# trailofbits/reverie

Measured on AMD Instinct MI355X. Metric: prover AND-gates/sec on GF(2) Bristol circuit; 1/2/4/8-GPU; proof bit-exact, higher is better.
Workload: dtype u32; 1 GPU; synthetic layered AND/XOR GF(2) circuit, 10027008 gates (5014185 AND), 4096 inputs, 153 layers x 65536, p_and=0.5, 256 reps x 8 players, 40 online; parallelism=reps/1, levels=163, compile_hint=RV_COMPILE_WHOLE_PROVER, gate_stream_bytes=334698564

## Files before the change

reverie_amd/csrc/gf2dev.h:

```cpp
#pragma once
#include <hip/hip_runtime.h>
#include <stdint.h>

namespace rv {

__device__ __forceinline__ uint32_t smear01(uint32_t t) {
    uint32_t r;
    asm("v_lshlrev_b32 %0, 8, %1\n\tv_sub_u32 %0, %0, %1" : "=&v"(r) : "v"(t));
    return r;
}
__device__ __forceinline__ uint32_t recon32(uint32_t t) {
    t ^= t >> 4;
    t ^= t >> 2;
    t ^= t >> 1;
    t &= 0x01010101u;
    return smear01(t);
}

__device__ __forceinline__ uint32_t expand4(uint32_t n) {
    const uint32_t t = (n | (n << 7) | (n << 14) | (n << 21)) & 0x01010101u;
    return smear01(t);
}
__device__ __forceinline__ uint32_t compress4(uint32_t x) {
    const uint32_t y = x & 0x08040201u;
    return (y | (y >> 8) | (y >> 16) | (y >> 24)) & 0xFu;
}
__device__ __forceinline__ uint32_t load_bits(const uint8_t* base, size_t row, uint32_t NQ, uint32_t q) {
    return expand4(((uint32_t)base[row * (NQ >> 1) + (q >> 1)] >> (4 * (q & 1))) & 0xFu);
}
__device__ __forceinline__ uint32_t pair_swap(uint32_t v) {
    return (uint32_t)__builtin_amdgcn_mov_dpp((int)v, 0xB1, 0xF, 0xF, true);
}
__device__ __forceinline__ void store_bits(uint8_t* base, size_t row, uint32_t NQ, uint32_t q, uint32_t smeared) {
    const uint32_t n = compress4(smeared);
    const uint32_t other = pair_swap(n);
    if (!(q & 1)) base[row * (NQ >> 1) + (q >> 1)] = (uint8_t)(n | (other << 4));
}

}
```

reverie_amd/csrc/internal.h:

```cpp
#pragma once
#include <hip/hip_runtime.h>
#include <stddef.h>
#include <stdint.h>

#include "../../include/reverie_amd.h"

namespace rv {


constexpr int RV_LIN_K = 3;
struct Gate {
    uint32_t op;
    uint32_t dst;
    uint32_t m;
    uint32_t eo;
    uint32_t ep;
    uint32_t x;
    uint32_t a[RV_LIN_K], b[RV_LIN_K];
};

enum GateOp : uint32_t {
    G_INPUT = 0,
    G_XORK,
    G_MUL,
// ... 14 lines not shown
    uint32_t m;
    uint32_t m2;
    uint64_t eo;
    uint64_t ep;
    uint32_t x;
    uint32_t xc;
    uint64_t imm;
    uint32_t am, bm;
};
constexpr uint32_t G64_MASK_ROW = 0x80000000u;

enum Gate64Op : uint32_t {
    G64_INPUT = 0, G64_ADD, G64_SUB, G64_ADDC, G64_SUBC, G64_MULC, G64_MUL, G64_ASSERT, G64_RANDOM, G64_CONST, G64_B2A
};

struct Interp64Params {
    uint32_t R;
    uint64_t* wmask;
    uint64_t* wcorr;
    const uint64_t* masks;
    uint64_t* on;
    uint64_t* pre;
    uint64_t on_words, pre_words;
    const uint64_t* wit;
    const uint8_t* omit;
    const uint64_t* sup_in;
    const uint64_t* sup_corr;
    const uint64_t* sup_rec;
    uint32_t sup_r;
    const uint8_t* corr2;
    const uint32_t* masks2;
    uint32_t NQ;
    int* err;
};

enum Mode : int { MODE_PROVE = 0, MODE_VERIFY = 1, MODE_PROVE_V = 2,  MODE_VERIFY_C = 4 };
constexpr int RV_DEV_ZERO_CHECK = 0x100;

struct InterpParams {
    uint32_t NQ;
    uint32_t* rows;
    uint8_t* corr;
    uint32_t* on;
    uint8_t* pre;
    uint8_t* vclr;
    uint64_t* vc;
    const uint8_t* wit;
    const uint32_t* on_mask;
    const uint32_t* sup_in;
    const uint32_t* sup_corr;
    const uint32_t* sup_rec;
    uint32_t sup_nq;
    int* err;
};

void set_device_lds_limit(size_t bytes);
size_t device_lds_limit();

struct EvalParams {
    uint32_t B, W;
    uint32_t* val;
    const uint32_t* win;
    uint64_t* v64;
    const uint64_t* wz;
    uint64_t wz_stride;
    uint32_t* n_failed;
    uint32_t* first2;
    uint32_t* first64;
};
struct WireForm {
    uint32_t b[RV_LIN_K];
    uint32_t c;
};
void launch_eval_level(hipStream_t st, const EvalParams& p, const Gate* d_gates, uint32_t lo, uint32_t n2, const Gate64* d_gates64, uint32_t lo64,
                       uint32_t n64);
struct LevelRange;
void launch_eval_walk(hipStream_t st, const EvalParams& p, const Gate* d_gates, const LevelRange* d_lr, const Gate64* d_gates64, const uint32_t* d_ls64,
                      uint32_t n_levels, uint32_t S, uint32_t threads);
void launch_eval_wit(hipStream_t st, const uint8_t* d_wit , uint32_t n, uint32_t B, uint32_t W, uint32_t* d_out );
void launch_eval_out(hipStream_t st, const EvalParams& p, const WireForm* d_forms, uint32_t n_gf2, const uint32_t* d_ssa64, uint32_t n_z64,
                     uint8_t* d_out2 , uint64_t* d_out64 );

struct EvalFold {
    const uint32_t* rec2;
    const uint64_t* op2;
    const uint32_t* rec64;
    const uint64_t* op64;
    uint32_t n2, n64;
    uint64_t op_base;
    uint64_t* first_op;
    uint64_t* total;
};
void launch_eval_fold(hipStream_t st, const EvalParams& p, const EvalFold& f);
void launch_eval_stream_out(hipStream_t st, const EvalParams& p, uint32_t n_gf2, uint32_t n_z64, uint32_t b0, uint32_t nb, uint8_t* d_out2,
                            uint64_t* d_out64);

void launch_expand_seeds(hipStream_t st, const uint8_t* d_seeds, uint32_t n_reps, uint8_t* d_keys );
constexpr uint32_t RK_BYTES = 208;
constexpr uint32_t RK_AREAS = 13;
constexpr uint64_t RV_MAX_CTR_BLOCKS = 1ull << 24;
void launch_key_schedule(hipStream_t st, const uint8_t* d_keys, uint32_t n_slots, uint8_t* d_rkbytes );
void launch_setup_keys(hipStream_t st, const uint8_t* d_seeds, uint32_t NQ, uint8_t* d_keys, uint8_t* d_rkbytes, uint32_t* d_rk, uint32_t* d_img);
void launch_bitslice_rk(hipStream_t st, const uint8_t* d_rkbytes, uint32_t NQ, uint32_t* d_rk );
void launch_aes_gf2_masks(hipStream_t st, const uint32_t* d_rk, const uint32_t* d_keep, uint32_t NQ, uint64_t first_block,
                          uint64_t n_blocks, uint32_t* d_masks);
bool aes_col4_supports(uint32_t NQ);
// ... 150 lines not shown
```

reverie_amd/csrc/kernels.hip:

```cpp
#include <stdlib.h>

#include <algorithm>

#include "b3.h"
#include "gf2dev.h"
#include "internal.h"
#include "launch.h"

namespace rv {

static size_t g_device_lds_limit = 160 * 1024;
void set_device_lds_limit(size_t bytes) { g_device_lds_limit = bytes; }
size_t device_lds_limit() { return g_device_lds_limit; }


__device__ __forceinline__ uint32_t gather_rows(const uint32_t* rows, const uint32_t* ids, uint32_t NQ, uint32_t q) {
    uint32_t v = 0;
#pragma unroll
    for (int i = 0; i < RV_LIN_K; i++) v ^= rows[(size_t)ids[i] * NQ + q];
    return v;
}
__device__ __forceinline__ uint32_t gather_corr_byte(const uint8_t* corr, const uint32_t* ids, uint32_t NQ, uint32_t o) {
    uint32_t v = 0;
#pragma unroll
// ... 26 lines not shown
    v |= (uint32_t)__builtin_amdgcn_update_dpp(0, (int)v, 0x111, 0xF, 0xF, true);
    v |= (uint32_t)__builtin_amdgcn_update_dpp(0, (int)v, 0x112, 0xF, 0xF, true);
    v |= (uint32_t)__builtin_amdgcn_update_dpp(0, (int)v, 0x114, 0xF, 0xF, true);
    if (q == 7 || q == 15) ((uint32_t*)(vc + row))[q >> 3] = v;
}
constexpr bool is_verify(int mode) { return mode == MODE_VERIFY || mode == MODE_VERIFY_C; }

#ifndef RV_COH_LDROW
#define RV_COH_LDROW 1
#endif
#ifndef RV_COH_STROW
#define RV_COH_STROW 1
#endif
#ifndef RV_COH_V
#define RV_COH_V 1
#endif
template <int COH>
__device__ __forceinline__ uint32_t ld_row(const uint32_t* p) {
    if (COH && RV_COH_LDROW) return __hip_atomic_load(const_cast<uint32_t*>(p), __ATOMIC_RELAXED, __HIP_MEMORY_SCOPE_AGENT);
    return *p;
}
template <int COH>
__device__ __forceinline__ void st_row(uint32_t* p, uint32_t v) {
    if (COH == 1 && RV_COH_STROW)
        __hip_atomic_store(p, v, __ATOMIC_RELAXED, __HIP_MEMORY_SCOPE_AGENT);
    else
        *p = v;
}
template <int COH>
__device__ __forceinline__ uint32_t ld_v(const uint8_t* p) {
    if (COH && RV_COH_V) return __hip_atomic_load(const_cast<uint8_t*>(p), __ATOMIC_RELAXED, __HIP_MEMORY_SCOPE_AGENT);
    return *p;
}
template <int COH>
__device__ __forceinline__ void st_v(uint8_t* p, uint8_t v) {
    if (COH == 1 && RV_COH_V)
        __hip_atomic_store(p, v, __ATOMIC_RELAXED, __HIP_MEMORY_SCOPE_AGENT);
    else
        *p = v;
}
template <int COH>
__device__ __forceinline__ uint32_t gather_rows_c(const uint32_t* rows, const uint32_t* ids, uint32_t NQ, uint32_t q) {
    uint32_t v = 0;
#pragma unroll
    for (int i = 0; i < RV_LIN_K; i++) v ^= ld_row<COH>(&rows[(size_t)ids[i] * NQ + q]);
    return v;
}
template <int COH>
__device__ __forceinline__ uint32_t gather_vclr_c(const uint8_t* vclr, const uint32_t* ids) {
    uint32_t v = 0;
#pragma unroll
    for (int i = 0; i < RV_LIN_K; i++) v ^= ld_v<COH>(&vclr[ids[i]]);
    return v;
}

template <int MODE, int COH = 0>
__device__ __forceinline__ void interp_one_impl(const Gate& g, const InterpParams& p, uint32_t NQ, uint32_t q, uint32_t onm) {
    switch (g_op(g)) {
    case G_INPUT: {
        const uint32_t lam = p.rows[(size_t)g.m * NQ + q];
        uint32_t corr;
        if (!is_verify(MODE)) {
            const uint32_t w = p.wit[g.x] ? 0xFFFFFFFFu : 0u;
            corr = w ^ recon32(lam);
        } else {
            corr = onm ? (p.sup_in[(size_t)g.x * p.sup_nq + q] & onm) : 0u;
        }
        if (!is_verify(MODE) || onm) p.on[(size_t)g.eo * NQ + q] = corr;
        if (MODE == MODE_PROVE_V) {
            if (q == 0) st_v<COH>(&p.vclr[g.dst], p.wit[g.x] ? 1 : 0);
        } else if (MODE == MODE_VERIFY_C) {
            vc_store(p.vc, g.dst, q, corr);
        } else {
            store_bits(p.corr, g.dst, NQ, q, corr);
        }
        break;
    }
    case G_XORK: {
        st_row<COH>(&p.rows[(size_t)g.dst * NQ + q], gather_rows_c<COH>(p.rows, g.a, NQ, q) ^ gather_rows_c<COH>(p.rows, g.b, NQ, q));
        if (MODE == MODE_PROVE_V) {
            if (q == 0) st_v<COH>(&p.vclr[g.dst], (uint8_t)((g_ca(g) ^ gather_vclr_c<COH>(p.vclr, g.a) ^ gather_vclr_c<COH>(p.vclr, g.b)) & 1u));
            break;
        }
        if (MODE == MODE_VERIFY_C) {
            if (q == 0) p.vc[g.dst] = gather_vc(p.vc, g.a) ^ gather_vc(p.vc, g.b) ^ (g_ca(g) ? ~0ull : 0ull);
            break;
        }
        if (!(q & 1)) {
            const size_t h = NQ >> 1, o = q >> 1;
            const uint32_t c = (g_ca(g) ? 0xFFu : 0u) ^ gather_corr_byte(p.corr, g.a, NQ, o) ^ gather_corr_byte(p.corr, g.b, NQ, o);
            p.corr[(size_t)g.dst * h + o] = (uint8_t)c;
        }
        break;
    }
    case G_RANDOM: {
        if (MODE == MODE_VERIFY_C) {
            if (q == 0) p.vc[g.dst] = 0;
            break;
        }
        if (!(q & 1)) p.corr[(size_t)g.dst * (NQ >> 1) + (q >> 1)] = 0;
        break;
    }
    case G_MUL: {
        const uint32_t lx = gather_rows_c<COH>(p.rows, g.a, NQ, q), ly = gather_rows_c<COH>(p.rows, g.b, NQ, q);
        const uint32_t lab = p.rows[(size_t)g.m * NQ + q], lnew = p.rows[(size_t)(g.m + 1) * NQ + q];
        const uint32_t a = recon32(lx), b = recon32(ly), c = recon32(lab);
// ... 80 lines not shown
}

#ifndef RV_B3_RPL
#define RV_B3_RPL 4
#endif
#ifndef RV_INTERP_UNROLL
#define RV_INTERP_UNROLL 4
#endif
#ifndef RV_INTERP_UNROLL_SMALL
#define RV_INTERP_UNROLL_SMALL 2
#endif
#ifndef RV_INTERP_UNROLL_MID
#define RV_INTERP_UNROLL_MID 4
#endif
#ifndef RV_INTERP_UNROLL_FAST
#define RV_INTERP_UNROLL_FAST 4
#endif
#ifndef RV_INTERP_UXOR_FAST
#define RV_INTERP_UXOR_FAST 0
#endif
__host__ __device__ constexpr int interp_unroll(int NQ, bool general = true) {
    return NQ >= 64 ? (general ? RV_INTERP_UNROLL : RV_INTERP_UNROLL_FAST) : NQ >= 32 ? RV_INTERP_UNROLL_MID : RV_INTERP_UNROLL_SMALL;
}

struct PfPlan {
    uint32_t dist;
    uint32_t rem;
    uint32_t n[2][4];
    uint32_t start[2][4];
};
template <uint32_t STEP>
__device__ __forceinline__ const Gate* pf_target(const Gate* __restrict__ gates, const PfPlan& pf, uint32_t t) {
    uint32_t tt = t + pf.dist;
#pragma unroll
    for (int k = 0; k < 2; k++) {
#pragma unroll
        for (int c = 0; c < 4; c++) {
            if (tt < pf.n[k][c]) return gates + pf.start[k][c] + tt * STEP;
            tt -= pf.n[k][c];
        }
        tt += pf.rem;
    }
    return nullptr;
}
template <uint32_t STEP>
__device__ __forceinline__ uint32_t pf_touch(const Gate* g, uint32_t lane) {
    constexpr uint32_t BYTES = STEP * (uint32_t)sizeof(Gate), NL = (BYTES + 127) / 128;
    uint32_t v = 0;
    if (g && lane <= NL) v = *(const uint32_t*)((const char*)g + (lane < NL ? lane * 128 : BYTES - 4));
    return v;
}
__device__ __forceinline__ void pf_sink(uint32_t v) { asm volatile("" ::"v"(v)); }

template <int MODE, int NQ, int U, int KA, int KB, int COH = 0>
__device__ __forceinline__ void mulU(const Gate* __restrict__ gates, uint32_t g0, const InterpParams& p, uint32_t sub, uint32_t q,
                                     uint32_t onm, const Gate* pf = nullptr) {
    constexpr uint32_t GPW = 64 / NQ, H = NQ / 2;
    const bool on_wr = !is_verify(MODE) || ((__ballot(onm != 0) >> ((sub * NQ + q) & ~7u)) & 0xFFull) != 0;
    Gate g[U];
#pragma unroll
    for (int u = 0; u < U; u++) g[u] = gates[g0 + u * GPW + sub];
    uint32_t lx[U], ly[U], lab[U], lnew[U], bx[U], by[U], sc[U], sr[U];
    uint32_t ra[U][KA], ca[U][KA], rb[U][KB], cb[U][KB];
    const uint32_t* const vc32 = (const uint32_t*)p.vc + ((q >> 3) & 1u);
#pragma unroll
    for (int u = 0; u < U; u++) {
        const int na = (int)g_na(g[u]), nb = (int)g_nb(g[u]);
#pragma unroll
        for (int i = 0; i < KA; i++) {
            ra[u][i] = 0;
            ca[u][i] = 0;
            if (i == 0 || i < na) {
                ra[u][i] = ld_row<COH>(&p.rows[(size_t)g[u].a[i] * NQ + q]);
                ca[u][i] = MODE == MODE_VERIFY_C ? vc32[2 * (size_t)g[u].a[i]]
                                                 : MODE == MODE_PROVE_V ? ld_v<COH>(&p.vclr[g[u].a[i]]) : p.corr[(size_t)g[u].a[i] * H + (q >> 1)];
            }
        }
#pragma unroll
        for (int i = 0; i < KB; i++) {
            rb[u][i] = 0;
            cb[u][i] = 0;
            if (i == 0 || i < nb) {
                rb[u][i] = ld_row<COH>(&p.rows[(size_t)g[u].b[i] * NQ + q]);
                cb[u][i] = MODE == MODE_VERIFY_C ? vc32[2 * (size_t)g[u].b[i]]
                                                 : MODE == MODE_PROVE_V ? ld_v<COH>(&p.vclr[g[u].b[i]]) : p.corr[(size_t)g[u].b[i] * H + (q >> 1)];
            }
        }
        lab[u] = __builtin_nontemporal_load(&p.rows[(size_t)g[u].m * NQ + q]);
        lnew[u] = p.rows[(size_t)(g[u].m + 1) * NQ + q];
        if (is_verify(MODE)) {
            sc[u] = sr[u] = 0;
            if (onm) {
                sc[u] = p.sup_corr[(size_t)g[u].ep * p.sup_nq + q];
                sr[u] = p.sup_rec[(size_t)g[u].x * p.sup_nq + q];
            }
        }
    }
    const uint32_t pfv = pf_touch<U * GPW>(pf, sub * NQ + q);
#pragma unroll
    for (int u = 0; u < U; u++) {
        lx[u] = ra[u][0];
        bx[u] = ca[u][0];
        ly[u] = rb[u][0];
        by[u] = cb[u][0];
#pragma unroll
        for (int i = 1; i < KA; i++) {
            lx[u] ^= ra[u][i];
            bx[u] ^= ca[u][i];
        }
#pragma unroll
        for (int i = 1; i < KB; i++) {
            ly[u] ^= rb[u][i];
            by[u] ^= cb[u][i];
        }
    }
#pragma unroll
    for (int u = 0; u < U; u++) {
        const uint32_t a = recon32(lx[u]), b = recon32(ly[u]), c = recon32(lab[u]);
        uint32_t cx, cy;
        const uint32_t vx = (bx[u] ^ g_ca(g[u])) & 1u, vy = (by[u] ^ g_cb(g[u])) & 1u;
        if (MODE == MODE_PROVE_V) {
            cx = a ^ (vx ? 0xFFFFFFFFu : 0u);
            cy = b ^ (vy ? 0xFFFFFFFFu : 0u);
        } else if (MODE == MODE_VERIFY_C) {
            cx = expand4(q < 16 ? (bx[u] >> (4 * (q & 7))) & 0xFu : 0u) ^ (g_ca(g[u]) ? 0xFFFFFFFFu : 0u);
            cy = expand4(q < 16 ? (by[u] >> (4 * (q & 7))) & 0xFu : 0u) ^ (g_cb(g[u]) ? 0xFFFFFFFFu : 0u);
        } else {
            cx = expand4((bx[u] >> (4 * (q & 1))) & 0xFu) ^ (g_ca(g[u]) ? 0xFFFFFFFFu : 0u);
            cy = expand4((by[u] >> (4 * (q & 1))) & 0xFu) ^ (g_cb(g[u]) ? 0xFFFFFFFFu : 0u);
        }
        uint32_t delta = (a & b) ^ c;
        uint32_t s = (ly[u] & cx) ^ (lx[u] & cy) ^ lab[u] ^ lnew[u];
        uint32_t r = 0;
        if (MODE == MODE_PROVE) {
            r = recon32(s);
        } else if (is_verify(MODE)) {
            delta = (sc[u] & onm) | (delta & ~onm);
            s ^= sr[u];
            r = recon32(s) & onm;
        }
        if (!is_verify(MODE) || on_wr) __builtin_nontemporal_store(s, &p.on[(size_t)g[u].eo * NQ + q]);
        store_bits(p.pre, g[u].ep, NQ, q, delta);
        if (MODE == MODE_PROVE_V) {
            if (q == 0) st_v<COH>(&p.vclr[g[u].dst], (uint8_t)(vx & vy));
        } else if (MODE == MODE_VERIFY_C) {
            vc_store(p.vc, g[u].dst, q, r ^ delta ^ (cx & cy));
        } else {
            store_bits(p.corr, g[u].dst, NQ, q, r ^ delta ^ (cx & cy));
        }
    }
    pf_sink(pfv);
}

template <int MODE, int NQ, int U, int N, int COH = 0>
__device__ __forceinline__ void xorU(const Gate* __restrict__ gates, uint32_t g0, const InterpParams& p, uint32_t sub, uint32_t q,
                                     const Gate* pf = nullptr) {
    constexpr uint32_t GPW = 64 / NQ, H = NQ / 2;
    Gate g[U];
#pragma unroll
    for (int u = 0; u < U; u++) g[u] = gates[g0 + u * GPW + sub];
    uint32_t x[U], bx[U], rr[U][N], cc[U][N];
#pragma unroll
    for (int u = 0; u < U; u++) {
        const int na = (int)g_na(g[u]), nb = (int)g_nb(g[u]);
#pragma unroll
        for (int i = 0; i < N; i++) {
            const uint32_t id = (N == 2) ? g[u].a[i] : (i < RV_LIN_K ? g[u].a[i] : g[u].b[i - RV_LIN_K]);
            rr[u][i] = 0;
            cc[u][i] = 0;
            if (N == 2 || (i < RV_LIN_K ? i < na : i - RV_LIN_K < nb)) {
                rr[u][i] = ld_row<COH>(&p.rows[(size_t)id * NQ + q]);
                if (MODE == MODE_PROVE_V) {
                    if (q == 0) cc[u][i] = ld_v<COH>(&p.vclr[id]);
                } else if (MODE == MODE_VERIFY_C) {
                    if (q < 2) cc[u][i] = ((const uint32_t*)p.vc)[2 * (size_t)id + q];
                } else if (q < H) {
                    cc[u][i] = p.corr[(size_t)id * H + q];
                }
            }
        }
    }
    const uint32_t pfv = pf_touch<U * GPW>(pf, sub * NQ + q);
#pragma unroll
    for (int u = 0; u < U; u++) {
        x[u] = 0;
        bx[u] = 0;
#pragma unroll
        for (int i = 0; i < N; i++) {
            x[u] ^= rr[u][i];
            bx[u] ^= cc[u][i];
        }
    }
#pragma unroll
    for (int u = 0; u < U; u++) {
        st_row<COH>(&p.rows[(size_t)g[u].dst * NQ + q], x[u]);
        if (MODE == MODE_PROVE_V) {
            if (q == 0) st_v<COH>(&p.vclr[g[u].dst], (uint8_t)((bx[u] ^ g_ca(g[u])) & 1u));
        } else if (MODE == MODE_VERIFY_C) {
            if (q < 2) ((uint32_t*)p.vc)[2 * (size_t)g[u].dst + q] = bx[u] ^ (g_ca(g[u]) ? 0xFFFFFFFFu : 0u);
        } else if (q < H) {
            p.corr[(size_t)g[u].dst * H + q] = (uint8_t)(bx[u] ^ (g_ca(g[u]) ? 0xFFu : 0u));
        }
    }
    pf_sink(pfv);
}

template <int MODE>
__device__ __forceinline__ void interp_one(const Gate& g, const InterpParams& p, uint32_t NQ, uint32_t q, uint32_t onm) {
    interp_one_impl<MODE>(g, p, NQ, q, onm);
}

template <int MODE, int NQ, bool ROTATE, bool GENERAL = true, bool PF = false, int UXOR = 0, int COH = 0>
__device__ __forceinline__ void run_level(const Gate* __restrict__ gates, const LevelRange& r, const InterpParams& p, uint32_t wave,
                                          uint32_t n_waves, uint32_t lane, uint32_t onm, const Gate* pf_gates = nullptr,
                                          const PfPlan* pf = nullptr) {
    constexpr uint32_t GPW = 64 / NQ;
    const uint32_t q = lane % NQ, sub = lane / NQ;
    constexpr int U = interp_unroll(NQ, GENERAL);
    constexpr int UX = UXOR ? UXOR : U;
    static_assert(!PF || UX == U, "the prefetch plan assumes one step size");
    uint32_t slot = 0;
    auto my = [&](uint32_t used) { return ROTATE ? (wave + n_waves - used % n_waves) % n_waves : wave; };
    const uint32_t begin[5] = {r.lo, r.mul11, r.mul, r.xor2, r.xork}, end[5] = {r.mul11, r.mul, r.xor2, r.xork, r.hi};
    uint32_t rest[5];
#pragma unroll
    for (int c = 0; c < 4; c++) {
        const uint32_t STEP = (uint32_t)(c >= 2 ? UX : U) * GPW;
        const uint32_t n_full = (!GENERAL && (c == 1 || c == 3)) ? 0u : (end[c] - begin[c]) / STEP;
        rest[c] = begin[c] + n_full * STEP;
        for (uint32_t g0 = begin[c] + my(slot) * STEP; g0 < rest[c]; g0 += n_waves * STEP) {
            const Gate* t = nullptr;
            if (PF && pf->dist) t = pf_target<U * GPW>(pf_gates, *pf, slot + (g0 - begin[c]) / STEP);
            if (c == 0) mulU<MODE, NQ, U, 1, 1, COH>(gates, g0, p, sub, q, onm, t);
            if (c == 1 && GENERAL) mulU<MODE, NQ, U, RV_LIN_K, RV_LIN_K, COH>(gates, g0, p, sub, q, onm, t);
            if (c == 2) xorU<MODE, NQ, UX, 2, COH>(gates, g0, p, sub, q, t);
            if (c == 3 && GENERAL) xorU<MODE, NQ, UX, 2 * RV_LIN_K, COH>(gates, g0, p, sub, q, t);
        }
        slot += n_full;
    }
    rest[4] = begin[4];
    uint32_t cum[6];
    cum[0] = 0;
#pragma unroll
    for (int c = 0; c < 5; c++) cum[c + 1] = cum[c] + (end[c] - rest[c] + GPW - 1) / GPW;
    for (uint32_t t = my(slot); t < cum[5]; t += n_waves) {
        uint32_t c0 = rest[0], e0 = end[0], base = 0;
#pragma unroll
        for (int c = 1; c < 5; c++)
            if (t >= cum[c]) c0 = rest[c], e0 = end[c], base = cum[c];
        const uint32_t gi = c0 + (t - base) * GPW + sub;
        if (gi < e0) interp_one_impl<MODE, COH>(gates[gi], p, NQ, q, onm);
    }
}

template <int MODE, int NQ, bool GENERAL>
__global__ __launch_bounds__(256, MODE == MODE_VERIFY_C ? (GENERAL ? 4 : 7) : (GENERAL || NQ != 64) ? 1 : 8) void k_interp_full(const Gate* __restrict__ gates, LevelRange r, InterpParams p, PfPlan pf) {
    __builtin_amdgcn_s_setprio(1);
    const uint32_t lane = threadIdx.x & 63;
    const uint32_t wave = __builtin_amdgcn_readfirstlane((blockIdx.x * blockDim.x + threadIdx.x) >> 6);
    const uint32_t n_waves = gridDim.x * (blockDim.x >> 6);
    const uint32_t onm = (is_verify(MODE)) ? p.on_mask[lane % NQ] : 0u;
    constexpr int UXL = (!GENERAL && NQ == 64) ? RV_INTERP_UXOR_FAST : 0;
    constexpr bool PFL = UXL == 0 || UXL == interp_unroll(NQ, GENERAL);
    run_level<MODE, NQ, true, GENERAL, PFL, UXL>(gates, r, p, wave, n_waves, lane, onm, gates, &pf);
}

template <int MODE, int NQ>
__global__ __launch_bounds__(256) void k_interp_full_b(const Gate* __restrict__ gates, LevelRange r, const InterpParams* __restrict__ pp) {
    const InterpParams p = pp[blockIdx.y];
    const uint32_t lane = threadIdx.x & 63;
    const uint32_t wave = __builtin_amdgcn_readfirstlane((blockIdx.x * blockDim.x + threadIdx.x) >> 6);
    const uint32_t n_waves = gridDim.x * (blockDim.x >> 6);
    const uint32_t onm = (is_verify(MODE)) ? p.on_mask[lane % NQ] : 0u;
    run_level<MODE, NQ, true>(gates, r, p, wave, n_waves, lane, onm);
}

static bool level_is_general(const LevelRange& r) { return (r.mul - r.mul11) + (r.xork - r.xor2) >= 64; }

static uint32_t pf_dist(int NQ) {
    static const int env = [] {
        const char* e = getenv("RV_PF_DIST");
        return e ? atoi(e) : -1;
    }();
    const uint32_t v = env >= 0 ? (uint32_t)env : (NQ == 64 ? 4096u : 0u);
    return v & ~31u;
}

template <int NQ>
static PfPlan make_pf_plan(const LevelRange& r, const LevelRange* next) {
    constexpr uint32_t GPW = 64 / NQ;
    PfPlan pf{};
    pf.dist = pf_dist(NQ);
    if (!pf.dist) return pf;
    const LevelRange* lr[2] = {&r, next};
    uint32_t total = 0;
    for (int k = 0; k < 2; k++) {
        if (!lr[k]) break;
        const LevelRange& x = *lr[k];
        const bool general = level_is_general(x);
        const uint32_t step = (uint32_t)interp_unroll(NQ, general) * GPW;
        const uint32_t begin[4] = {x.lo, x.mul11, x.mul, x.xor2}, end[4] = {x.mul11, x.mul, x.xor2, x.xork};
        for (int c = 0; c < 4; c++) {
            pf.start[k][c] = begin[c];
            pf.n[k][c] = (!general && (c == 1 || c == 3)) ? 0u : (end[c] - begin[c]) / step;
            if (k == 0) total += pf.n[k][c];
        }
    }
    pf.rem = total & 31u;
    return pf;
}

template <int NQ>
static void launch_interp_full(hipStream_t st, int mode, const Gate* d_gates, const LevelRange& r, const InterpParams& p,
                               const LevelRange* next) {
    constexpr uint32_t GPW = 64 / NQ;
    const bool general = level_is_general(r);
    const PfPlan pf = make_pf_plan<NQ>(r, next);
    const uint32_t u = (uint32_t)interp_unroll(NQ, general);
    uint64_t waves = ((uint64_t)(r.hi - r.lo) + u * GPW - 1) / (u * GPW);
    uint64_t blocks = (waves + 3) / 4;
    if (blocks > 4096) blocks = 4096;
    if (blocks < 1) blocks = 1;
    if (mode == MODE_PROVE_V) {
        if (general)
            hipLaunchKernelGGL((k_interp_full<MODE_PROVE_V, NQ, true>), dim3((unsigned)blocks), dim3(256), 0, st, d_gates, r, p, pf);
        else
            hipLaunchKernelGGL((k_interp_full<MODE_PROVE_V, NQ, false>), dim3((unsigned)blocks), dim3(256), 0, st, d_gates, r, p, pf);
    } else if (mode == MODE_PROVE) {
        if (general)
            hipLaunchKernelGGL((k_interp_full<MODE_PROVE, NQ, true>), dim3((unsigned)blocks), dim3(256), 0, st, d_gates, r, p, pf);
        else
            hipLaunchKernelGGL((k_interp_full<MODE_PROVE, NQ, false>), dim3((unsigned)blocks), dim3(256), 0, st, d_gates, r, p, pf);
    } else if (mode == MODE_VERIFY_C && NQ == 64) {
        if (general)
            hipLaunchKernelGGL((k_interp_full<NQ == 64 ? MODE_VERIFY_C : MODE_VERIFY, NQ, true>), dim3((unsigned)blocks), dim3(256), 0, st, d_gates, r, p, pf);
        else
            hipLaunchKernelGGL((k_interp_full<NQ == 64 ? MODE_VERIFY_C : MODE_VERIFY, NQ, false>), dim3((unsigned)blocks), dim3(256), 0, st, d_gates, r, p, pf);
    } else {
        if (general)
            hipLaunchKernelGGL((k_interp_full<MODE_VERIFY, NQ, true>), dim3((unsigned)blocks), dim3(256), 0, st, d_gates, r, p, pf);
        else
            hipLaunchKernelGGL((k_interp_full<MODE_VERIFY, NQ, false>), dim3((unsigned)blocks), dim3(256), 0, st, d_gates, r, p, pf);
    }
}


bool persist_general(const LevelRange* lr, size_t n_levels) {
    for (size_t l = 0; l < n_levels; l++)
        if (level_is_general(lr[l])) return true;
    return false;
}

constexpr uint32_t NARROW_MAX_LEVELS = 1024;
constexpr uint32_t NARROW_WIN = 1024;
template <int MODE, int NQT, bool LEAN = false>
__device__ __forceinline__ void interp_narrow_body(const Gate* __restrict__ gates, const LevelRange* __restrict__ level_range,
                                                   uint32_t l0, uint32_t l1, const InterpParams& p) {
    __shared__ LevelRange s_lr[NARROW_MAX_LEVELS];
    __shared__ __attribute__((aligned(16))) Gate s_g[NARROW_WIN];
    const uint32_t NQ = NQT ? (uint32_t)NQT : p.NQ;
    const uint32_t lane = threadIdx.x & 63, wave = threadIdx.x >> 6;
    const uint32_t onm = (is_verify(MODE)) ? p.on_mask[NQT ? lane % NQ : threadIdx.x % NQ] : 0u;
    const uint32_t n_lv = l1 - l0;
    {
        const uint32_t* src = (const uint32_t*)(level_range + l0);
        uint32_t* dst = (uint32_t*)s_lr;
        for (uint32_t i = threadIdx.x; i < n_lv * (uint32_t)(sizeof(LevelRange) / 4); i += 1024) dst[i] = src[i];
    }
    __syncthreads();
    const uint32_t g_end = s_lr[n_lv - 1].hi;
    uint32_t win_lo = s_lr[0].lo, win_hi = win_lo;
    for (uint32_t l = 0; l < n_lv; l++) {
        const LevelRange r = s_lr[l];
        if (r.hi > win_hi) {
            win_lo = r.lo;
            win_hi = (r.lo + NARROW_WIN < g_end) ? r.lo + NARROW_WIN : g_end;
            const uint4* src = (const uint4*)(gates + win_lo);
// ... 1606 lines not shown
```

reverie_amd/csrc/shard.inc:

```
struct HostTrace {
    bool on = false;
    std::chrono::steady_clock::time_point t0;
    std::vector<std::pair<const char*, double>> marks;
    void begin() {
        static const bool env = getenv("RV_BATCH_STATS") != nullptr;
        on = env;
        marks.clear();
        t0 = std::chrono::steady_clock::now();
    }
    void mark(const char* what) {
        if (on) marks.emplace_back(what, std::chrono::duration<double, std::milli>(std::chrono::steady_clock::now() - t0).count());
    }
};
static thread_local HostTrace g_ht;

struct EarlyRun {
    const EarlyPlan* plan = nullptr;
    uint8_t* d_ec = nullptr;
    uint8_t* h_ec = nullptr;
    size_t next = 0;
    size_t pumped = 0;
    std::vector<uint8_t> packed;
    uint32_t* box_dev = nullptr;
    volatile uint32_t* box = nullptr;
// ... 233 lines not shown
}

static const uint32_t* b3_empty_digest() {
    static const std::vector<uint32_t> empty = [] {
        b3::Hasher hs;
        uint8_t out[32];
        hs.finalize(out);
        std::vector<uint32_t> w(8);
        for (int k = 0; k < 8; k++) w[k] = (uint32_t)out[4 * k] | ((uint32_t)out[4 * k + 1] << 8) | ((uint32_t)out[4 * k + 2] << 16) | ((uint32_t)out[4 * k + 3] << 24);
        return w;
    }();
    return empty.data();
}

static int shard_run_alloc(rv_shard* s, InterpParams& p, Interp64Params& p64) {
    rv_ctx* ctx = s->ctx;
    const Compiled& cc = s->c->cc;
    int rc;
    if ((rc = dalloc(ctx, (size_t)cc.n_rows * (s->NQ / 2), &s->d_wires))) return rc;
    if ((rc = dalloc(ctx, (size_t)std::max<uint64_t>(cc.n_on, 1) * s->NQ, &s->d_on))) return rc;
    if ((rc = dalloc(ctx, (size_t)std::max<uint64_t>(cc.n_pre, 1) * (s->NQ / 2), &s->d_pre))) return rc;
    if (!s->d_err && (rc = dalloc(ctx, 1, &s->d_err))) return rc;
    const size_t cvw = b3_stream_scratch_words(std::max({cc.n_on, cc.n_pre, cc.on_words64 * 8, cc.pre_words64 * 8}), s->R);
    if ((rc = dalloc(ctx, cvw, &s->d_cv[0])) || (rc = dalloc(ctx, cvw, &s->d_cv[1]))) return rc;
    if (b3_pair_big_ok(cc.n_pre, cc.n_on, s->NQ, s->d_on_quads, s->n_on_quads)) {
        const size_t w2 = b3_stream_scratch_words(std::max(cc.n_on, cc.n_pre), s->R);
        if ((rc = dalloc(ctx, w2, &s->d_cv2[0])) || (rc = dalloc(ctx, w2, &s->d_cv2[1]))) return rc;
        s->extra.push_back(s->d_cv2[0]);
        s->extra.push_back(s->d_cv2[1]);
    }
    if ((rc = dalloc(ctx, (size_t)4 * s->R * 8, &s->d_dig))) return rc;
    if (!s->d_h && (rc = dalloc(ctx, (size_t)s->R * 32, &s->d_h))) return rc;
    const bool has64 = !cc.gates64.empty();
    if (has64) {
        if ((rc = dalloc(ctx, (size_t)cc.n_ssa64 * s->R * 8, &s->d_wmask64))) return rc;
        if (s->z64f && !s->d_keys64) {
            if ((rc = dalloc(ctx, (size_t)cc.n_ssa64, &s->d_v64))) return rc;
            HIPCHK(hipMemsetAsync(s->d_v64, 0, 8, ctx->stream));
        } else {
            if ((rc = dalloc(ctx, (size_t)cc.n_ssa64 * s->R, &s->d_wcorr64))) return rc;
            HIPCHK(rv::memset_async(s->d_wcorr64, 0, (size_t)s->R * 8, ctx->stream));
        }
        if ((rc = dalloc(ctx, (size_t)std::max<uint64_t>(cc.on_words64, 1) * s->R, &s->d_on64))) return rc;
        if ((rc = dalloc(ctx, (size_t)std::max<uint64_t>(cc.pre_words64, 1) * s->R, &s->d_pre64))) return rc;
        HIPCHK(rv::memset_async(s->d_wmask64, 0, (size_t)s->R * 64, ctx->stream));
    }
    hipStream_t sb = ctx->stream;
    s->dig64_filled = !g_recorder && cc.pre_words64 == 0 && cc.on_words64 == 0;
    launch_shard_init(sb, s->d_err, s->d_masks + (size_t)cc.zero_row * s->NQ, s->NQ,
                      s->d_wires + (size_t)cc.zero_row * (s->NQ / 2), s->NQ / 2, s->dig64_filled ? s->d_dig + 2 * (size_t)s->R * 8 : nullptr, 2 * s->R,
                      b3_empty_digest(), p.vclr ? p.vclr + cc.zero_row : nullptr);
    p.NQ = s->NQ;
    p.rows = s->d_masks;
    p.corr = s->d_wires;
    p.on = s->d_on;
    p.pre = s->d_pre;
    p.err = s->d_err;
    p64.R = s->R;
    p64.wmask = s->d_wmask64;
    p64.wcorr = s->d_wcorr64;
    p64.masks = s->d_masks64;
    p64.on = s->d_on64;
    p64.pre = s->d_pre64;
    p64.on_words = cc.on_words64;
    p64.pre_words = cc.pre_words64;
    p64.corr2 = s->d_wires;
    p64.masks2 = s->d_masks;
    p64.NQ = s->NQ;
    p64.err = s->d_err;
    return RV_OK;
}

static bool lds_run_fits_rows(uint32_t qs, uint32_t NQ) { return NQ % qs == 0 && (qs > 1 || NQ % 8 == 0); }

static bool lds_run_for_batch(const rv_circuit* c, size_t level, size_t batch) {
    if (c->lds_run_of_level[level] < 0) return false;
    const auto& pl = c->lds_runs[(size_t)c->lds_run_of_level[level]];
    const size_t limit = getenv("RV_LDS_BATCH_WGS") ? (size_t)atoll(getenv("RV_LDS_BATCH_WGS")) : 768;
    return batch * (RV_TOTAL_REPS / 4 / pl.qs) <= limit;
}

static std::atomic<uint64_t> g_overlap_commits{0};
extern "C" uint64_t rv_hook_overlap_commits(void) { return g_overlap_commits.load(std::memory_order_relaxed); }
static std::atomic<uint64_t> g_early_proofs{0};
extern "C" uint64_t rv_hook_early_proofs(void) { return g_early_proofs.load(std::memory_order_relaxed); }
static std::atomic<uint64_t> g_open_direct_proofs{0};
extern "C" uint64_t rv_hook_open_direct_proofs(void) { return g_open_direct_proofs.load(std::memory_order_relaxed); }
static std::atomic<uint64_t> g_verify_vc{0};
extern "C" uint64_t rv_hook_verify_vc_count(void) { return g_verify_vc.load(std::memory_order_relaxed); }

static void early_plan_build(const rv_circuit* c, EarlyPlan& P) {
    const Compiled& cc = c->cc;
    const uint64_t min_events = getenv("RV_EARLY_MIN") ? (uint64_t)atoll(getenv("RV_EARLY_MIN")) : (1ull << 21);
    const int n_chunks_env = getenv("RV_EARLY_CHUNKS") ? std::min(atoi(getenv("RV_EARLY_CHUNKS")), 255) : 4;
    auto reps_env = [](uint32_t dflt) -> uint32_t {
        const char* e = getenv("RV_EARLY_REPS");
        if (!e) return dflt;
        return (uint32_t)std::min(std::max(atoi(e), 0), (int)RV_TOTAL_REPS);
    };
    const size_t n_levels = cc.level_start.empty() ? 0 : cc.level_start.size() - 1;
    if (!cc.gates64.empty()) {
        const size_t n_lv64 = cc.level_start64.empty() ? 0 : cc.level_start64.size() - 1;
        const uint64_t min64 = getenv("RV_EARLY_MIN") ? min_events : (1ull << 17);
        if (cc.row_prg_base || cc.n_pre || cc.pre_words64 != cc.n_corr64 || cc.n_corr64 < min64 || (cc.n_corr64 & 1) || !n_lv64 || n_chunks_env < 1) return;
        std::vector<uint64_t> lo(n_lv64, UINT64_MAX);
        for (size_t l = 0; l < n_lv64; l++)
// ... 466 lines not shown
    auto fail = [&](int code) {
        rv_shard_destroy(s);
        return code;
    };
    const size_t seed_bytes = (size_t)s->R * 16;
    const bool stage_in = defer_sync && seed_bytes + cc.n_in <= rv_ctx::IN_STAGE_BYTES &&
                          (ctx->h_in || hipHostMalloc((void**)&ctx->h_in, rv_ctx::IN_STAGE_BYTES, hipHostMallocDefault) == hipSuccess);
    if (!stage_in) (void)hipGetLastError();
    if (stage_in) {
        if ((rc = dalloc(ctx, seed_bytes + std::max<size_t>(cc.n_in, 1), &s->d_seeds)) || (rc = dalloc(ctx, (size_t)s->R * 128, &s->d_keys))) return fail(rc);
        s->d_wit = s->d_seeds + seed_bytes;
        memcpy(ctx->h_in, seeds, seed_bytes);
        if (cc.n_in) memcpy(ctx->h_in + seed_bytes, wit_gf2, cc.n_in);
        if (hipMemcpyAsync(s->d_seeds, ctx->h_in, seed_bytes + cc.n_in, hipMemcpyHostToDevice, ctx->stream) != hipSuccess) return fail(RV_E_DEVICE);
    } else {
        if ((rc = dalloc(ctx, seed_bytes, &s->d_seeds)) || (rc = dalloc(ctx, (size_t)s->R * 128, &s->d_keys)) ||
            (rc = dalloc(ctx, std::max<size_t>(cc.n_in, 1), &s->d_wit)))
            return fail(rc);
        if (hipMemcpyAsync(s->d_seeds, seeds, seed_bytes, hipMemcpyHostToDevice, ctx->stream) != hipSuccess) return fail(RV_E_DEVICE);
        if (cc.n_in && hipMemcpyAsync(s->d_wit, wit_gf2, cc.n_in, hipMemcpyHostToDevice, ctx->stream) != hipSuccess) return fail(RV_E_DEVICE);
    }
    if (cc.n_in64) {
        if ((rc = dalloc(ctx, cc.n_in64, &s->d_wit64))) return fail(rc);
        if (hipMemcpyAsync(s->d_wit64, wit_z64, cc.n_in64 * 8, hipMemcpyHostToDevice, ctx->stream) != hipSuccess)
            return fail(RV_E_DEVICE);
    }
    static const bool vclr_on = [] {
        const char* e = getenv("RV_VCLR");
        return !e || atoi(e) != 0;
    }();
    const bool use_vclr = vclr_on && c->vclr_ok && (s->NQ == 64 || s->NQ == 32 || s->NQ == 16 || s->NQ == 8);
    s->z64f = c->z64f_ok && z64_fused_on() && z64_fused_supports(s->NQ) && !g_recorder;
    {
        const int ov_mode = getenv("RV_OVERLAP") ? atoi(getenv("RV_OVERLAP")) : 1;
        const uint64_t ov_min = getenv("RV_OVERLAP_MIN") ? strtoull(getenv("RV_OVERLAP_MIN"), nullptr, 0) : 8192;
        s->overlap = ov_mode != 0 && !g_recorder && aes_col4_supports(s->NQ) &&
                     cc.n_masks_pad / 128 >= ov_min;
    }
    ctx->phase(RV_PH_SETUP);
    ctx->count();
    s->keys_deferred = !g_recorder && s->R == 4 * s->NQ;
    if (!s->keys_deferred) launch_expand_seeds(ctx->stream, s->d_seeds, s->R, s->d_keys);
    {
        g_ht.mark("inputs");
        if ((rc = shard_setup_prg(s, nullptr))) return fail(rc);
        g_ht.mark("prg");
        if (ec) s->ec = ec;
        InterpParams p{};
        p.wit = s->d_wit;
        Interp64Params p64{};
        p64.wit = s->d_wit64;
        int mode = MODE_PROVE;
        if (use_vclr) {
            if ((rc = dalloc(ctx, (size_t)cc.n_rows, &s->d_vclr))) return fail(rc);
            p.vclr = s->d_vclr;
            mode = MODE_PROVE_V;
        }
        if ((rc = shard_run(s, mode, p, p64))) return fail(rc);
    }
    if ((rc = shard_join(s))) return fail(rc);
    if (defer_sync) {
        ctx->prof.calls++;
        *out = s;
        return RV_OK;
    }
    int err = 0;
    if (hipMemcpyAsync(&err, s->d_err, sizeof err, hipMemcpyDeviceToHost, ctx->stream) != hipSuccess) return fail(RV_E_DEVICE);
    hipError_t e = hipStreamSynchronize(ctx->stream);
    if (e != hipSuccess) {
        hip_fail(e, "hipStreamSynchronize", __FILE__, __LINE__);
        return fail(RV_E_DEVICE);
    }
    ctx->collect();
    ctx->prof.calls++;
    if (err) return fail(RV_E_WITNESS_INVALID);
    *out = s;
    return RV_OK;
}

extern "C" int rv_shard_digests_device(rv_shard* s, void** dptr) {
    if (!s || !dptr) return RV_E_ARG;
    *dptr = s->d_h;
    return RV_OK;
}

extern "C" int rv_shard_digests(rv_shard* s, uint8_t* out) {
    if (!s || !out) return RV_E_ARG;
    HIPCHK(hipMemcpyAsync(out, s->d_h, (size_t)s->R * 32, hipMemcpyDeviceToHost, s->ctx->stream));
    HIPCHK(hipStreamSynchronize(s->ctx->stream));
    return RV_OK;
}

extern "C" int rv_shard_digests_to_device(rv_shard* s, void* dst_device) {
    if (!s || !dst_device) return RV_E_ARG;
    HIPCHK(hipMemcpyAsync(dst_device, s->d_h, (size_t)s->R * 32, hipMemcpyDeviceToDevice, s->ctx->stream));
    HIPCHK(hipStreamSynchronize(s->ctx->stream));
    return RV_OK;
}

extern "C" int rv_hook_shard_stream_digests(rv_shard* s, uint8_t* out) {
    if (!s || !out) return RV_E_ARG;
    std::vector<uint32_t> tmp((size_t)4 * s->R * 8);
    HIPCHK(hipMemcpyAsync(tmp.data(), s->d_dig, tmp.size() * 4, hipMemcpyDeviceToHost, s->ctx->stream));
    HIPCHK(hipStreamSynchronize(s->ctx->stream));
    for (uint32_t r = 0; r < s->R; r++)
        for (int k = 0; k < 4; k++) memcpy(out + ((size_t)r * 4 + k) * 32, &tmp[((size_t)k * s->R + r) * 8], 32);
    return RV_OK;
// ... 2 lines not shown
```

Measured before the change: 1.002 billion AND gates/s.

## Use buffer loads/stores with 32-bit offsets and scalar vclr loads in interp kernel

Adds a UNI specialization of the NQ=64 non-general interpreter that addresses rows, corr, on, pre and vclr through AMD buffer resource descriptors with 32-bit offsets. It is enabled only when every array fits below 4 GiB. vclr bytes are read through the scalar constant address space as aligned words, and the vclr allocation is padded to a multiple of 4 bytes. The prove-path AND-gate maths is restructured to work on 0/1 parity bytes, so it skips the smear/compress round trips. The aim is to cut 64-bit address arithmetic, VGPR pressure and redundant vector loads. The cost is added specialization and reliance on the scalar-load assumption that vclr is uniform across the wave.

Result: no change. 1.007 billion AND gates/s, median of 6 (+0.5%).

```diff
diff --git a/reverie_amd/csrc/gf2dev.h b/reverie_amd/csrc/gf2dev.h
--- a/reverie_amd/csrc/gf2dev.h
+++ b/reverie_amd/csrc/gf2dev.h
@@ -9,13 +9,13 @@
     asm("v_lshlrev_b32 %0, 8, %1\n\tv_sub_u32 %0, %0, %1" : "=&v"(r) : "v"(t));
     return r;
 }
-__device__ __forceinline__ uint32_t recon32(uint32_t t) {
+__device__ __forceinline__ uint32_t parity01(uint32_t t) {
     t ^= t >> 4;
     t ^= t >> 2;
     t ^= t >> 1;
-    t &= 0x01010101u;
-    return smear01(t);
+    return t & 0x01010101u;
 }
+__device__ __forceinline__ uint32_t recon32(uint32_t t) { return smear01(parity01(t)); }
 
 __device__ __forceinline__ uint32_t expand4(uint32_t n) {
     const uint32_t t = (n | (n << 7) | (n << 14) | (n << 21)) & 0x01010101u;
@@ -25,6 +25,7 @@
     const uint32_t y = x & 0x08040201u;
     return (y | (y >> 8) | (y >> 16) | (y >> 24)) & 0xFu;
 }
+__device__ __forceinline__ uint32_t compress01(uint32_t t) { return (t | (t >> 7) | (t >> 14) | (t >> 21)) & 0xFu; }
 __device__ __forceinline__ uint32_t load_bits(const uint8_t* base, size_t row, uint32_t NQ, uint32_t q) {
     return expand4(((uint32_t)base[row * (NQ >> 1) + (q >> 1)] >> (4 * (q & 1))) & 0xFu);
 }
diff --git a/reverie_amd/csrc/internal.h b/reverie_amd/csrc/internal.h
--- a/reverie_amd/csrc/internal.h
+++ b/reverie_amd/csrc/internal.h
@@ -90,6 +90,7 @@
     const uint32_t* sup_rec;
     uint32_t sup_nq;
     int* err;
+    uint32_t below_4g;
 };
 
 void set_device_lds_limit(size_t bytes);
diff --git a/reverie_amd/csrc/kernels.hip b/reverie_amd/csrc/kernels.hip
--- a/reverie_amd/csrc/kernels.hip
+++ b/reverie_amd/csrc/kernels.hip
@@ -102,6 +102,19 @@
 #pragma unroll
     for (int i = 0; i < RV_LIN_K; i++) v ^= ld_v<COH>(&vclr[ids[i]]);
     return v;
+}
+
+__device__ __forceinline__ __amdgpu_buffer_rsrc_t rsrc(const void* base) {
+    return __builtin_amdgcn_make_buffer_rsrc(const_cast<void*>(base), (short)0, (int)0xFFFFFFFFu, 0x00020000);
+}
+constexpr int BUF_NT = 2;
+__device__ __forceinline__ uint32_t lane_off(uint32_t v) {
+    asm("" : "+v"(v));
+    return v;
+}
+__device__ __forceinline__ uint32_t ld_v_scalar(const uint8_t* vclr, uint32_t id) {
+    const __attribute__((address_space(4))) uint32_t* w = (const __attribute__((address_space(4))) uint32_t*)(vclr + (id & ~3u));
+    return (*w >> (8 * (id & 3u))) & 1u;
 }
 
 template <int MODE, int COH = 0>
@@ -288,17 +301,38 @@
 }
 __device__ __forceinline__ void pf_sink(uint32_t v) { asm volatile("" ::"v"(v)); }
 
-template <int MODE, int NQ, int U, int KA, int KB, int COH = 0>
+template <int MODE, int NQ, int U, int KA, int KB, int COH = 0, bool UNI = false>
 __device__ __forceinline__ void mulU(const Gate* __restrict__ gates, uint32_t g0, const InterpParams& p, uint32_t sub, uint32_t q,
                                      uint32_t onm, const Gate* pf = nullptr) {
     constexpr uint32_t GPW = 64 / NQ, H = NQ / 2;
+    constexpr bool SA = UNI && NQ == 64 && COH == 0, SV = UNI && NQ == 64 && MODE == MODE_PROVE_V;
+    const uint32_t q4 = lane_off(4 * q), h = lane_off(q >> 1);
+    const __amdgpu_buffer_rsrc_t rs = rsrc(p.rows), rc = rsrc(p.corr);
+    auto row = [&](uint32_t id) -> uint32_t {
+        if (SA) return __builtin_amdgcn_raw_buffer_load_b32(rs, q4, id * (NQ * 4), 0);
+        return ld_row<COH>(&p.rows[(size_t)id * NQ + q]);
+    };
+    auto val = [&](uint32_t id) -> uint32_t {
+        if (MODE == MODE_VERIFY_C) return ((const uint32_t*)p.vc + ((q >> 3) & 1u))[2 * (size_t)id];
+        if (SV) return ld_v_scalar(p.vclr, id);
+        if (MODE == MODE_PROVE_V) return ld_v<COH>(&p.vclr[id]);
+        if (SA) return __builtin_amdgcn_raw_buffer_load_b8(rc, h, id * H, 0);
+        return p.corr[(size_t)id * H + (q >> 1)];
+    };
+    auto bits = [&](uint8_t* base, uint32_t r, uint32_t n) {
+        const uint32_t other = pair_swap(n);
+        if (q & 1) return;
+        if (SA)
+            __builtin_amdgcn_raw_buffer_store_b8((uint8_t)(n | (other << 4)), rsrc(base), h, r * H, 0);
+        else
+            base[(size_t)r * H + (q >> 1)] = (uint8_t)(n | (other << 4));
+    };
     const bool on_wr = !is_verify(MODE) || ((__ballot(onm != 0) >> ((sub * NQ + q) & ~7u)) & 0xFFull) != 0;
     Gate g[U];
 #pragma unroll
     for (int u = 0; u < U; u++) g[u] = gates[g0 + u * GPW + sub];
     uint32_t lx[U], ly[U], lab[U], lnew[U], bx[U], by[U], sc[U], sr[U];
     uint32_t ra[U][KA], ca[U][KA], rb[U][KB], cb[U][KB];
-    const uint32_t* const vc32 = (const uint32_t*)p.vc + ((q >> 3) & 1u);
 #pragma unroll
     for (int u = 0; u < U; u++) {
         const int na = (int)g_na(g[u]), nb = (int)g_nb(g[u]);
@@ -307,9 +341,8 @@
             ra[u][i] = 0;
             ca[u][i] = 0;
             if (i == 0 || i < na) {
-                ra[u][i] = ld_row<COH>(&p.rows[(size_t)g[u].a[i] * NQ + q]);
-                ca[u][i] = MODE == MODE_VERIFY_C ? vc32[2 * (size_t)g[u].a[i]]
-                                                 : MODE == MODE_PROVE_V ? ld_v<COH>(&p.vclr[g[u].a[i]]) : p.corr[(size_t)g[u].a[i] * H + (q >> 1)];
+                ra[u][i] = row(g[u].a[i]);
+                ca[u][i] = val(g[u].a[i]);
             }
         }
 #pragma unroll
@@ -317,13 +350,17 @@
             rb[u][i] = 0;
             cb[u][i] = 0;
             if (i == 0 || i < nb) {
-                rb[u][i] = ld_row<COH>(&p.rows[(size_t)g[u].b[i] * NQ + q]);
-                cb[u][i] = MODE == MODE_VERIFY_C ? vc32[2 * (size_t)g[u].b[i]]
-                                                 : MODE == MODE_PROVE_V ? ld_v<COH>(&p.vclr[g[u].b[i]]) : p.corr[(size_t)g[u].b[i] * H + (q >> 1)];
-            }
-        }
-        lab[u] = __builtin_nontemporal_load(&p.rows[(size_t)g[u].m * NQ + q]);
-        lnew[u] = p.rows[(size_t)(g[u].m + 1) * NQ + q];
+                rb[u][i] = row(g[u].b[i]);
+                cb[u][i] = val(g[u].b[i]);
+            }
+        }
+        if (SA) {
+            lab[u] = __builtin_amdgcn_raw_buffer_load_b32(rs, q4, g[u].m * (NQ * 4), BUF_NT);
+            lnew[u] = __builtin_amdgcn_raw_buffer_load_b32(rs, q4, (g[u].m + 1) * (NQ * 4), 0);
+        } else {
+            lab[u] = __builtin_nontemporal_load(&p.rows[(size_t)g[u].m * NQ + q]);
+            lnew[u] = p.rows[(size_t)(g[u].m + 1) * NQ + q];
+        }
         if (is_verify(MODE)) {
             sc[u] = sr[u] = 0;
             if (onm) {
@@ -352,12 +389,12 @@
     }
 #pragma unroll
     for (int u = 0; u < U; u++) {
-        const uint32_t a = recon32(lx[u]), b = recon32(ly[u]), c = recon32(lab[u]);
+        const uint32_t pa = parity01(lx[u]), pb = parity01(ly[u]), pc = parity01(lab[u]);
         uint32_t cx, cy;
         const uint32_t vx = (bx[u] ^ g_ca(g[u])) & 1u, vy = (by[u] ^ g_cb(g[u])) & 1u;
         if (MODE == MODE_PROVE_V) {
-            cx = a ^ (vx ? 0xFFFFFFFFu : 0u);
-            cy = b ^ (vy ? 0xFFFFFFFFu : 0u);
+            cx = smear01(pa) ^ (vx ? 0xFFFFFFFFu : 0u);
+            cy = smear01(pb) ^ (vy ? 0xFFFFFFFFu : 0u);
         } else if (MODE == MODE_VERIFY_C) {
             cx = expand4(q < 16 ? (bx[u] >> (4 * (q & 7))) & 0xFu : 0u) ^ (g_ca(g[u]) ? 0xFFFFFFFFu : 0u);
             cy = expand4(q < 16 ? (by[u] >> (4 * (q & 7))) & 0xFu : 0u) ^ (g_cb(g[u]) ? 0xFFFFFFFFu : 0u);
@@ -365,33 +402,46 @@
             cx = expand4((bx[u] >> (4 * (q & 1))) & 0xFu) ^ (g_ca(g[u]) ? 0xFFFFFFFFu : 0u);
             cy = expand4((by[u] >> (4 * (q & 1))) & 0xFu) ^ (g_cb(g[u]) ? 0xFFFFFFFFu : 0u);
         }
-        uint32_t delta = (a & b) ^ c;
+        const uint32_t d01 = (pa & pb) ^ pc;
         uint32_t s = (ly[u] & cx) ^ (lx[u] & cy) ^ lab[u] ^ lnew[u];
-        uint32_t r = 0;
-        if (MODE == MODE_PROVE) {
-            r = recon32(s);
-        } else if (is_verify(MODE)) {
-            delta = (sc[u] & onm) | (delta & ~onm);
+        if (!is_verify(MODE)) {
+            if (SA)
+                __builtin_amdgcn_raw_buffer_store_b32(s, rsrc(p.on), q4, g[u].eo * (NQ * 4), BUF_NT);
+            else
+                __builtin_nontemporal_store(s, &p.on[(size_t)g[u].eo * NQ + q]);
+            bits(p.pre, g[u].ep, compress01(d01));
+            if (MODE == MODE_PROVE_V) {
+                if (q == 0) {
+                    if (SA)
+                        __builtin_amdgcn_raw_buffer_store_b8((uint8_t)(vx & vy), rsrc(p.vclr), 0, g[u].dst, 0);
+                    else
+                        st_v<COH>(&p.vclr[g[u].dst], (uint8_t)(vx & vy));
+                }
+            } else {
+                bits(p.corr, g[u].dst, compress01(parity01(s) ^ d01 ^ (cx & cy & 0x01010101u)));
+            }
+        } else {
+            const uint32_t delta = (sc[u] & onm) | (smear01(d01) & ~onm);
             s ^= sr[u];
-            r = recon32(s) & onm;
-        }
-        if (!is_verify(MODE) || on_wr) __builtin_nontemporal_store(s, &p.on[(size_t)g[u].eo * NQ + q]);
-        store_bits(p.pre, g[u].ep, NQ, q, delta);
-        if (MODE == MODE_PROVE_V) {
-            if (q == 0) st_v<COH>(&p.vclr[g[u].dst], (uint8_t)(vx & vy));
-        } else if (MODE == MODE_VERIFY_C) {
-            vc_store(p.vc, g[u].dst, q, r ^ delta ^ (cx & cy));
-        } else {
-            store_bits(p.corr, g[u].dst, NQ, q, r ^ delta ^ (cx & cy));
+            const uint32_t r = recon32(s) & onm;
+            if (on_wr) __builtin_nontemporal_store(s, &p.on[(size_t)g[u].eo * NQ + q]);
+            store_bits(p.pre, g[u].ep, NQ, q, delta);
+            if (MODE == MODE_VERIFY_C)
+                vc_store(p.vc, g[u].dst, q, r ^ delta ^ (cx & cy));
+            else
+                store_bits(p.corr, g[u].dst, NQ, q, r ^ delta ^ (cx & cy));
         }
     }
     pf_sink(pfv);
 }
 
-template <int MODE, int NQ, int U, int N, int COH = 0>
+template <int MODE, int NQ, int U, int N, int COH = 0, bool UNI = false>
 __device__ __forceinline__ void xorU(const Gate* __restrict__ gates, uint32_t g0, const InterpParams& p, uint32_t sub, uint32_t q,
                                      const Gate* pf = nullptr) {
     constexpr uint32_t GPW = 64 / NQ, H = NQ / 2;
+    constexpr bool SA = UNI && NQ == 64 && COH == 0, SV = UNI && NQ == 64 && MODE == MODE_PROVE_V;
+    const uint32_t q4 = lane_off(4 * q);
+    const __amdgpu_buffer_rsrc_t rs = rsrc(p.rows);
     Gate g[U];
 #pragma unroll
     for (int u = 0; u < U; u++) g[u] = gates[g0 + u * GPW + sub];
@@ -405,8 +455,10 @@
             rr[u][i] = 0;
             cc[u][i] = 0;
             if (N == 2 || (i < RV_LIN_K ? i < na : i - RV_LIN_K < nb)) {
-                rr[u][i] = ld_row<COH>(&p.rows[(size_t)id * NQ + q]);
-                if (MODE == MODE_PROVE_V) {
+                rr[u][i] = SA ? __builtin_amdgcn_raw_buffer_load_b32(rs, q4, id * (NQ * 4), 0) : ld_row<COH>(&p.rows[(size_t)id * NQ + q]);
+                if (SV) {
+                    cc[u][i] = ld_v_scalar(p.vclr, id);
+                } else if (MODE == MODE_PROVE_V) {
                     if (q == 0) cc[u][i] = ld_v<COH>(&p.vclr[id]);
                 } else if (MODE == MODE_VERIFY_C) {
                     if (q < 2) cc[u][i] = ((const uint32_t*)p.vc)[2 * (size_t)id + q];
@@ -429,9 +481,17 @@
     }
 #pragma unroll
     for (int u = 0; u < U; u++) {
-        st_row<COH>(&p.rows[(size_t)g[u].dst * NQ + q], x[u]);
+        if (SA)
+            __builtin_amdgcn_raw_buffer_store_b32(x[u], rs, q4, g[u].dst * (NQ * 4), 0);
+        else
+            st_row<COH>(&p.rows[(size_t)g[u].dst * NQ + q], x[u]);
         if (MODE == MODE_PROVE_V) {
-            if (q == 0) st_v<COH>(&p.vclr[g[u].dst], (uint8_t)((bx[u] ^ g_ca(g[u])) & 1u));
+            if (q == 0) {
+                if (SA)
+                    __builtin_amdgcn_raw_buffer_store_b8((uint8_t)((bx[u] ^ g_ca(g[u])) & 1u), rsrc(p.vclr), 0, g[u].dst, 0);
+                else
+                    st_v<COH>(&p.vclr[g[u].dst], (uint8_t)((bx[u] ^ g_ca(g[u])) & 1u));
+            }
         } else if (MODE == MODE_VERIFY_C) {
             if (q < 2) ((uint32_t*)p.vc)[2 * (size_t)g[u].dst + q] = bx[u] ^ (g_ca(g[u]) ? 0xFFFFFFFFu : 0u);
         } else if (q < H) {
@@ -446,7 +506,7 @@
     interp_one_impl<MODE>(g, p, NQ, q, onm);
 }
 
-template <int MODE, int NQ, bool ROTATE, bool GENERAL = true, bool PF = false, int UXOR = 0, int COH = 0>
+template <int MODE, int NQ, bool ROTATE, bool GENERAL = true, bool PF = false, int UXOR = 0, int COH = 0, bool UNI = false>
 __device__ __forceinline__ void run_level(const Gate* __restrict__ gates, const LevelRange& r, const InterpParams& p, uint32_t wave,
                                           uint32_t n_waves, uint32_t lane, uint32_t onm, const Gate* pf_gates = nullptr,
                                           const PfPlan* pf = nullptr) {
@@ -467,10 +527,10 @@
         for (uint32_t g0 = begin[c] + my(slot) * STEP; g0 < rest[c]; g0 += n_waves * STEP) {
             const Gate* t = nullptr;
             if (PF && pf->dist) t = pf_target<U * GPW>(pf_gates, *pf, slot + (g0 - begin[c]) / STEP);
-            if (c == 0) mulU<MODE, NQ, U, 1, 1, COH>(gates, g0, p, sub, q, onm, t);
-            if (c == 1 && GENERAL) mulU<MODE, NQ, U, RV_LIN_K, RV_LIN_K, COH>(gates, g0, p, sub, q, onm, t);
-            if (c == 2) xorU<MODE, NQ, UX, 2, COH>(gates, g0, p, sub, q, t);
-            if (c == 3 && GENERAL) xorU<MODE, NQ, UX, 2 * RV_LIN_K, COH>(gates, g0, p, sub, q, t);
+            if (c == 0) mulU<MODE, NQ, U, 1, 1, COH, UNI>(gates, g0, p, sub, q, onm, t);
+            if (c == 1 && GENERAL) mulU<MODE, NQ, U, RV_LIN_K, RV_LIN_K, COH, UNI>(gates, g0, p, sub, q, onm, t);
+            if (c == 2) xorU<MODE, NQ, UX, 2, COH, UNI>(gates, g0, p, sub, q, t);
+            if (c == 3 && GENERAL) xorU<MODE, NQ, UX, 2 * RV_LIN_K, COH, UNI>(gates, g0, p, sub, q, t);
         }
         slot += n_full;
     }
@@ -489,7 +549,7 @@
     }
 }
 
-template <int MODE, int NQ, bool GENERAL>
+template <int MODE, int NQ, bool GENERAL, bool UNI = false>
 __global__ __launch_bounds__(256, MODE == MODE_VERIFY_C ? (GENERAL ? 4 : 7) : (GENERAL || NQ != 64) ? 1 : 8) void k_interp_full(const Gate* __restrict__ gates, LevelRange r, InterpParams p, PfPlan pf) {
     __builtin_amdgcn_s_setprio(1);
     const uint32_t lane = threadIdx.x & 63;
@@ -498,7 +558,7 @@
     const uint32_t onm = (is_verify(MODE)) ? p.on_mask[lane % NQ] : 0u;
     constexpr int UXL = (!GENERAL && NQ == 64) ? RV_INTERP_UXOR_FAST : 0;
     constexpr bool PFL = UXL == 0 || UXL == interp_unroll(NQ, GENERAL);
-    run_level<MODE, NQ, true, GENERAL, PFL, UXL>(gates, r, p, wave, n_waves, lane, onm, gates, &pf);
+    run_level<MODE, NQ, true, GENERAL, PFL, UXL, 0, UNI>(gates, r, p, wave, n_waves, lane, onm, gates, &pf);
 }
 
 template <int MODE, int NQ>
@@ -557,8 +617,11 @@
     uint64_t blocks = (waves + 3) / 4;
     if (blocks > 4096) blocks = 4096;
     if (blocks < 1) blocks = 1;
+    const bool uni = NQ == 64 && p.below_4g && !general;
     if (mode == MODE_PROVE_V) {
-        if (general)
+        if (uni)
+            hipLaunchKernelGGL((k_interp_full<MODE_PROVE_V, NQ, false, NQ == 64>), dim3((unsigned)blocks), dim3(256), 0, st, d_gates, r, p, pf);
+        else if (general)
             hipLaunchKernelGGL((k_interp_full<MODE_PROVE_V, NQ, true>), dim3((unsigned)blocks), dim3(256), 0, st, d_gates, r, p, pf);
         else
             hipLaunchKernelGGL((k_interp_full<MODE_PROVE_V, NQ, false>), dim3((unsigned)blocks), dim3(256), 0, st, d_gates, r, p, pf);
diff --git a/reverie_amd/csrc/shard.inc b/reverie_amd/csrc/shard.inc
--- a/reverie_amd/csrc/shard.inc
+++ b/reverie_amd/csrc/shard.inc
@@ -309,6 +309,8 @@
                       b3_empty_digest(), p.vclr ? p.vclr + cc.zero_row : nullptr);
     p.NQ = s->NQ;
     p.rows = s->d_masks;
+    p.below_4g = (uint64_t)cc.n_rows * s->NQ * 4 <= 0xFFFFFFFFull && std::max<uint64_t>(cc.n_on, 1) * s->NQ * 4 <= 0xFFFFFFFFull &&
+                 std::max<uint64_t>(cc.n_pre, 1) * (s->NQ / 2) <= 0xFFFFFFFFull;
     p.corr = s->d_wires;
     p.on = s->d_on;
     p.pre = s->d_pre;
@@ -881,7 +883,7 @@
         p64.wit = s->d_wit64;
         int mode = MODE_PROVE;
         if (use_vclr) {
-            if ((rc = dalloc(ctx, (size_t)cc.n_rows, &s->d_vclr))) return fail(rc);
+            if ((rc = dalloc(ctx, ((size_t)cc.n_rows + 3) & ~(size_t)3, &s->d_vclr))) return fail(rc);
             p.vclr = s->d_vclr;
             mode = MODE_PROVE_V;
         }
```
